# Orbis-Tertius/tiny-ram-halo2

Hardware: AMD Instinct MI355X
Metric: Pallas MSM pairs/s @ 2^24 + Fp NTT elems/s @ 2^22; 1/2/4/8 MI355X (higher is better)
Workload: dtype u255 (255-bit modular integers as 9 x 29/30-bit limbs in i32 / i64 lanes)

## Files before the change

tiny-ram-halo2_amd/csrc/msm.hip:

```cpp
#include <stdlib.h>
#include <string.h>

#include "ctx.h"
#include "devmem.h"
#include "curve_q4.h"
#include "hostcombine.h"
#include "hosthelper.h"
#include "hostplan.h"

namespace trh {

namespace {

using hostplan::MAX_C; using hostplan::MAX_C_FIXED; using hostplan::MSM_TILE; using hostplan::SMALL_C; using hostplan::SMALL_MAX_N;
using hostplan::PART_TILE; using hostplan::BIN_THREADS; using hostplan::BIN_PER_MAX; using hostplan::BIN_CAP_MAX; using hostplan::RANGE_BLOCK;
using hostplan::HEAVY_PIECES; using hostplan::SP_LISTS; using hostplan::SP_CNT; using hostplan::SP_PAD; using hostplan::SP_PARTS; using hostplan::SP_MAX_CHUNK;
using hostplan::num_windows;
static_assert(sizeof(XYZZMem) == hostplan::XYZZ_BYTES && sizeof(XYZZzMem) == hostplan::RAW_POINT_BYTES, "point sizes of the plan's scratch layout");
constexpr u32 SIGN_BIT = 0x80000000u;

template <class SF>
__global__ void __launch_bounds__(256) msm_recode_kernel(const uint4* __restrict__ scalars, size_t n, int mont, int c, int W,
                                                         u32* __restrict__ digits, u32* __restrict__ bin_counts, int k2, u32 nbins, int use_lds, size_t sstride,
                                                         int one_row ,
                                                         const uint4* __restrict__ tails ,
                                                         unsigned char* __restrict__ tile_flags ,
                                                         u32 tile_log, u32 tiles) {
    const size_t z = blockIdx.z;
    const u32 rows = one_row ? 1u : (u32)W;
    scalars += z * sstride * 2; digits += z * (size_t)W * n; bin_counts += z * (size_t)rows * nbins;
    extern __shared__ u32 lhist[];
    const u32 total = rows * nbins;
    if (use_lds) {
        for (u32 k = threadIdx.x; k < total; k += blockDim.x) lhist[k] = 0;
        __syncthreads();
    }
    const u32 mask = (1u << c) - 1u, half = 1u << (c - 1);
    for (size_t i = (size_t)blockIdx.x * blockDim.x + threadIdx.x; i < n; i += (size_t)gridDim.x * blockDim.x) {
        const uint4* src = (tails && i == n - 1) ? tails + 2 * z : scalars + 2 * i;
        uint4 lo = src[0], hi = src[1];
        u32 w[8] = {lo.x, lo.y, lo.z, lo.w, hi.x, hi.y, hi.z, hi.w};
        if (mont) fe_store(fe_from_mont(fe_load<SF>(w)), w);
        u32 carry = 0;
        for (int j = 0; j < W; ++j) {
            u32 raw = (w[0] & mask) + carry;
#pragma unroll
            for (int k = 0; k < 7; ++k) w[k] = (w[k] >> c) | (w[k + 1] << (32 - c));
            w[7] >>= c;
            u32 bucket, sign = 0;
            if (raw > half) { bucket = (1u << c) - raw; carry = 1; sign = SIGN_BIT; }
            else { bucket = raw; carry = 0; }
            digits[(size_t)j * n + i] = bucket ? (bucket | sign) : 0u;
            if (tile_flags) {
                const unsigned long long nz = __ballot(bucket != 0);
                const size_t slot = (size_t)j * n + i;
                const u32 lane = threadIdx.x & 63u;
                if (bucket && ((nz & ((1ull << lane) - 1ull)) == 0ull || (slot & (((size_t)1 << tile_log) - 1)) < 64))
                    tile_flags[z * tiles + (slot >> tile_log)] = 1;
            }
            if (bucket) {
                const u32 bin = (bucket - 1u) >> k2, row = one_row ? 0u : (u32)j;
                if (use_lds) atomicAdd(&lhist[row * nbins + bin], 1u);
                else atomicAdd(&bin_counts[(size_t)row * nbins + bin], 1u);
            }
        }
    }
    if (use_lds) {
        __syncthreads();
        for (u32 k = threadIdx.x; k < total; k += blockDim.x) {
            const u32 v = lhist[k];
            if (v) atomicAdd(&bin_counts[k], v);
        }
    }
}

struct ZeroRanges { uint4* p[4]; u32 n16[4]; };
__global__ void __launch_bounds__(256) msm_zero_ranges_kernel(const ZeroRanges z) {
    const uint4 zero = make_uint4(0, 0, 0, 0);
#pragma unroll
    for (int k = 0; k < 4; ++k)
        for (u32 i = blockIdx.x * blockDim.x + threadIdx.x; i < z.n16[k]; i += gridDim.x * blockDim.x) z.p[k][i] = zero;
}

__global__ void __launch_bounds__(1024) msm_offsets_kernel(u32* __restrict__ counts, u32* __restrict__ starts, u32 nb1, u32* __restrict__ oversize, u32 bin_cap,
                                                           u32* __restrict__ totals ) {
    const size_t z = blockIdx.z;
    counts += z * (size_t)gridDim.x * nb1; starts += z * (size_t)gridDim.x * nb1;
    __shared__ u32 part[1024];
    const int j = blockIdx.x, t = threadIdx.x;
    u32* cnt = counts + (size_t)j * nb1;
    u32* st = starts + (size_t)j * nb1;
    const u32 per = (nb1 + 1023u) / 1024u;
    const u32 lo = t * per < nb1 ? t * per : nb1, hi = (lo + per < nb1) ? lo + per : nb1;
    u32 sum = 0, biggest = 0;
    for (u32 b = lo; b < hi; ++b) { const u32 v = cnt[b]; sum += v; biggest = v > biggest ? v : biggest; }
    if (oversize && biggest > bin_cap) atomicMax(oversize + z * gridDim.x + blockIdx.x, biggest);
    part[t] = sum;
    __syncthreads();
    for (int off = 1; off < 1024; off <<= 1) {
        u32 v = (t >= off) ? part[t - off] : 0;
        __syncthreads();
        part[t] += v;
        __syncthreads();
    }
    if (totals && t == 1023) totals[z * gridDim.x + blockIdx.x] = part[1023];
    u32 run = part[t] - sum;
    for (u32 b = lo; b < hi; ++b) {
        u32 cv = cnt[b];
        st[b] = run;
        cnt[b] = run;
        run += cv;
    }
}

constexpr int PART_THREADS = 1024;
__global__ void __launch_bounds__(PART_THREADS) msm_partition_kernel(const u32* __restrict__ digits, u32* __restrict__ bin_cursor,
                                                                     u32* __restrict__ parted, size_t n, int k2, u32 nbins, int idx_bits,
                                                                     const unsigned char* __restrict__ tile_flags ) {
    const size_t z = blockIdx.z;
    if (tile_flags && !tile_flags[z * gridDim.x + blockIdx.x]) return;
    digits += z * (size_t)gridDim.y * n; parted += z * (size_t)gridDim.y * n; bin_cursor += z * (size_t)gridDim.y * nbins;
    extern __shared__ u32 lds[];
    u32* stage = lds;
    u32* cnt = lds + PART_TILE;
    u32* lbase = cnt + nbins;
    u32* gbase = lbase + nbins;
    __shared__ u32 scan[PART_THREADS];
    const int j = blockIdx.y;
    const size_t t0 = (size_t)blockIdx.x * PART_TILE;
    const size_t t1 = t0 + PART_TILE < n ? t0 + PART_TILE : n;
    const u32* dg = digits + (size_t)j * n;
    for (u32 k = threadIdx.x; k < nbins; k += blockDim.x) cnt[k] = 0;
    __syncthreads();
    constexpr int PER = PART_TILE / PART_THREADS;
    u32 mine[PER];
#pragma unroll
    for (int q = 0; q < PER; ++q) {
        const size_t i = t0 + threadIdx.x + (size_t)q * PART_THREADS;
        mine[q] = i < t1 ? dg[i] : 0u;
    }
#pragma unroll
    for (int q = 0; q < PER; ++q) {
        const u32 b = mine[q] & ~SIGN_BIT;
        if (b) atomicAdd(&cnt[(b - 1u) >> k2], 1u);
    }
    __syncthreads();
    {
        const u32 per = (nbins + PART_THREADS - 1) / PART_THREADS;
        const u32 lo = threadIdx.x * per < nbins ? threadIdx.x * per : nbins, hi = lo + per < nbins ? lo + per : nbins;
        u32 sum = 0;
        for (u32 k = lo; k < hi; ++k) sum += cnt[k];
        scan[threadIdx.x] = sum;
        __syncthreads();
        for (int off = 1; off < PART_THREADS; off <<= 1) {
            const u32 v = ((int)threadIdx.x >= off) ? scan[threadIdx.x - off] : 0;
            __syncthreads();
            scan[threadIdx.x] += v;
            __syncthreads();
        }
        u32 run = scan[threadIdx.x] - sum;
        for (u32 k = lo; k < hi; ++k) {
            const u32 v = cnt[k];
            lbase[k] = run;
            gbase[k] = v ? atomicAdd(&bin_cursor[(size_t)j * nbins + k], v) : 0u;
            run += v;
        }
    }
    __syncthreads();
    for (u32 k = threadIdx.x; k < nbins; k += blockDim.x) cnt[k] = 0;
    __syncthreads();
    const u32 low_mask = (1u << k2) - 1u;
#pragma unroll
    for (int q = 0; q < PER; ++q) {
        const u32 e = mine[q];
        const u32 b = e & ~SIGN_BIT;
        if (b) {
            const u32 bm = b - 1u, bin = bm >> k2;
            const u32 r = atomicAdd(&cnt[bin], 1u);
            stage[lbase[bin] + r] = (u32)(t0 + threadIdx.x + (size_t)q * PART_THREADS) | ((bm & low_mask) << idx_bits) | (e & SIGN_BIT);
        }
    }
    __syncthreads();
    u32* out = parted + (size_t)j * n;
    const u32 wave = threadIdx.x >> 6, lane = threadIdx.x & 63u;
    for (u32 bin = wave; bin < nbins; bin += PART_THREADS / 64) {
        const u32 c = cnt[bin], lb = lbase[bin], gb = gbase[bin];
        for (u32 k = lane; k < c; k += 64) out[gb + k] = stage[lb + k];
    }
}

constexpr int BS_CHUNK = 8192;
constexpr int BS_THREADS = 512;

__device__ __forceinline__ u32 bin_of_position(const u32* __restrict__ bin_ends, u32 nbins, u32 pos) {
    u32 lo = 0, hi = nbins;
    while (lo < hi) {
        const u32 mid = (lo + hi) >> 1;
        if (bin_ends[mid] > pos) hi = mid; else lo = mid + 1;
    }
    return lo;
}

template <bool SCATTER>
__global__ void __launch_bounds__(BS_THREADS) msm_bucket_pass_kernel(const u32* __restrict__ parted, const u32* __restrict__ bin_starts,
                                                                     const u32* __restrict__ bin_ends, u32* __restrict__ bucket_cnt ,
                                                                     u32* __restrict__ sorted, size_t n, int k2, u32 nbins, int idx_bits, u32 nbk,
                                                                     const u32* __restrict__ oversize) {
    const size_t z = blockIdx.z;
    {
        const size_t Wz = gridDim.y;
        parted += z * Wz * n; sorted += z * Wz * n; bin_starts += z * Wz * nbins; bin_ends += z * Wz * nbins;
        bucket_cnt += z * Wz * (nbk + 1);
    }
    if (oversize && oversize[z * gridDim.y + blockIdx.y] == 0u) return;
    __shared__ u32 cnt[128], tbase[128], gbase[128];
    __shared__ u32 stage[SCATTER ? BS_CHUNK : 1];
    const int j = blockIdx.y;
    const u32* bs = bin_starts + (size_t)j * nbins;
    const u32* be = bin_ends + (size_t)j * nbins;
    const u32 total = be[nbins - 1];
    const u32 c0 = blockIdx.x * BS_CHUNK;
    if (c0 >= total) return;
    const u32 c1 = c0 + BS_CHUNK < total ? c0 + BS_CHUNK : total;
    const u32 nsub = 1u << k2, low_mask = nsub - 1u, idx_mask = (1u << idx_bits) - 1u;
    const u32* src = parted + (size_t)j * n;
    u32* dst = sorted + (size_t)j * n;
    u32* bc = bucket_cnt + (size_t)j * (nbk + 1);
    const u32 wave = threadIdx.x >> 6, lane = threadIdx.x & 63u;
    for (u32 bin = bin_of_position(be, nbins, c0); bin < nbins; ++bin) {
        const u32 lo = bs[bin] > c0 ? bs[bin] : c0;
        if (lo >= c1) break;
        const u32 hi = be[bin] < c1 ? be[bin] : c1;
        if (hi <= lo) continue;
        if (hi - lo <= 64u) {
            if (threadIdx.x < hi - lo) {
                const u32 e = src[lo + threadIdx.x];
                u32* cell = &bc[(bin << k2) + ((e >> idx_bits) & low_mask) + 1u];
                if (!SCATTER) atomicAdd(cell, 1u);
                else dst[atomicAdd(cell, 1u)] = (e & idx_mask) | (e & SIGN_BIT);
            }
            continue;
        }
        if (threadIdx.x < 128) cnt[threadIdx.x] = 0;
        __syncthreads();
        for (u32 i = lo + threadIdx.x; i < hi; i += blockDim.x) atomicAdd(&cnt[(src[i] >> idx_bits) & low_mask], 1u);
        __syncthreads();
        if (!SCATTER) {
            if (threadIdx.x < nsub && cnt[threadIdx.x]) atomicAdd(&bc[(bin << k2) + threadIdx.x + 1u], cnt[threadIdx.x]);
        } else {
            if (threadIdx.x == 0) {
                u32 r = 0;
                for (u32 k = 0; k < nsub; ++k) { tbase[k] = r; r += cnt[k]; }
            }
            if (threadIdx.x < nsub) {
                const u32 v = cnt[threadIdx.x];
                gbase[threadIdx.x] = v ? atomicAdd(&bc[(bin << k2) + threadIdx.x + 1u], v) : 0u;
            }
            __syncthreads();
            if (threadIdx.x < 128) cnt[threadIdx.x] = 0;
            __syncthreads();
            for (u32 i = lo + threadIdx.x; i < hi; i += blockDim.x) {
                const u32 e = src[i];
                const u32 sub = (e >> idx_bits) & low_mask;
                const u32 r = atomicAdd(&cnt[sub], 1u);
                stage[tbase[sub] + r] = (e & idx_mask) | (e & SIGN_BIT);
            }
            __syncthreads();
            for (u32 sub = wave; sub < nsub; sub += BS_THREADS / 64) {
                const u32 c = cnt[sub], sb = tbase[sub], gb = gbase[sub];
                for (u32 k = lane; k < c; k += 64) dst[gb + k] = stage[sb + k];
            }
        }
        __syncthreads();
    }
}

template <int PER>
__global__ void __launch_bounds__(BIN_THREADS) msm_bin_sort_kernel(const u32* __restrict__ parted, const u32* __restrict__ bin_starts, const u32* __restrict__ bin_ends,
                                                                   u32* __restrict__ sorted, u32* __restrict__ starts, u32* __restrict__ ends, size_t n, int k2, u32 nbins,
                                                                   int idx_bits, u32 nbk, const u32* __restrict__ oversize) {
    if (oversize[(size_t)blockIdx.z * gridDim.y + blockIdx.y] != 0u) return;
    extern __shared__ u32 bstage[];
    __shared__ u32 cnt[128], tbase[128], wave0_total;
    const size_t z = blockIdx.z, Wz = gridDim.y;
    const int j = blockIdx.y;
    const u32 bin = blockIdx.x;
    const size_t wrow = z * Wz + j;
    const u32 lo = bin_starts[wrow * nbins + bin], hi = bin_ends[wrow * nbins + bin];
    const u32 count = hi - lo;
    const u32 nsub = 1u << k2, low_mask = nsub - 1u, idx_mask = (1u << idx_bits) - 1u;
    const u32* src = parted + wrow * n + lo;
    u32* dst = sorted + wrow * n + lo;
    const u32 lane = threadIdx.x & 63u;
    if (threadIdx.x < 128) cnt[threadIdx.x] = 0;
    __syncthreads();
    u32 mine[PER];
#pragma unroll
    for (int q = 0; q < PER; ++q) {
        const u32 i = threadIdx.x + (u32)q * BIN_THREADS;
        mine[q] = (u32)q * BIN_THREADS < count ? src[i < count ? i : 0u] : 0u;
    }
#pragma unroll
    for (int q = 0; q < PER; ++q)
        if (threadIdx.x + (u32)q * BIN_THREADS < count) atomicAdd(&cnt[(mine[q] >> idx_bits) & low_mask], 1u);
    __syncthreads();
    u32 v = 0, x = 0;
    if (threadIdx.x < 128) {
        v = threadIdx.x < nsub ? cnt[threadIdx.x] : 0u;
        x = v;
#pragma unroll
        for (int off = 1; off < 64; off <<= 1) {
            const u32 y = __shfl_up(x, off, 64);
            if ((int)lane >= off) x += y;
        }
        if (threadIdx.x == 63) wave0_total = x;
    }
    __syncthreads();
    if (threadIdx.x < 128) {
        const u32 excl = x - v + (threadIdx.x >= 64 ? wave0_total : 0u);
        tbase[threadIdx.x] = excl;
        cnt[threadIdx.x] = 0;
        if (threadIdx.x < nsub) {
            const size_t b = wrow * (nbk + 1) + ((size_t)bin << k2) + threadIdx.x + 1u;
            starts[b] = lo + excl;
            ends[b] = lo + excl + v;
        }
        if (bin == 0 && threadIdx.x == 0) { starts[wrow * (nbk + 1)] = 0; ends[wrow * (nbk + 1)] = 0; }
    }
    __syncthreads();
#pragma unroll
    for (int q = 0; q < PER; ++q) {
        if (threadIdx.x + (u32)q * BIN_THREADS < count) {
            const u32 e = mine[q];
            const u32 sub = (e >> idx_bits) & low_mask;
            const u32 r = atomicAdd(&cnt[sub], 1u);
            bstage[tbase[sub] + r] = (e & idx_mask) | (e & SIGN_BIT);
        }
    }
    __syncthreads();
#pragma unroll
    for (int q = 0; q < PER; ++q) {
        const u32 i = threadIdx.x + (u32)q * BIN_THREADS;
        if (i < count) mine[q] = bstage[i];
    }
#pragma unroll
    for (int q = 0; q < PER; ++q) {
        const u32 i = threadIdx.x + (u32)q * BIN_THREADS;
        if (i < count) dst[i] = mine[q];
    }
}

__global__ void __launch_bounds__(RANGE_BLOCK) msm_bucket_block_sums_kernel(const u32* __restrict__ bucket_cnt, u32* __restrict__ block_sums, u32 nbk,
                                                                            const u32* __restrict__ oversize) {
    if (oversize && oversize[(size_t)blockIdx.z * gridDim.y + blockIdx.y] == 0u) return;
    __shared__ u32 part[RANGE_BLOCK / 64];
    const size_t z = blockIdx.z, Wz = gridDim.y;
    const u32 nb1 = nbk + 1, b = blockIdx.x * RANGE_BLOCK + threadIdx.x;
    u32 v = b < nb1 ? bucket_cnt[(z * Wz + blockIdx.y) * nb1 + b] : 0u;
#pragma unroll
    for (int off = 32; off > 0; off >>= 1) v += __shfl_down(v, off, 64);
    if ((threadIdx.x & 63) == 0) part[threadIdx.x >> 6] = v;
    __syncthreads();
    if (threadIdx.x == 0) {
        u32 t = 0;
        for (int k = 0; k < RANGE_BLOCK / 64; ++k) t += part[k];
        block_sums[(z * Wz + blockIdx.y) * gridDim.x + blockIdx.x] = t;
    }
}
__global__ void __launch_bounds__(RANGE_BLOCK) msm_bucket_ranges_kernel(u32* __restrict__ bucket_cnt, const u32* __restrict__ block_sums, u32* __restrict__ starts,
                                                                        u32* __restrict__ ends, u32 nbk, const u32* __restrict__ oversize) {
// ... 666 lines not shown
        if ((int)threadIdx.x < st) sh[threadIdx.x] = xyzzz_add(sh[threadIdx.x], sh[threadIdx.x + st]);
        __syncthreads();
    }
    if (threadIdx.x == 0) store_raw(&part[z * SP_PARTS + g], sh[0]);
}

template <class BF>
__global__ void __launch_bounds__(64) msm_unit_final_kernel(const u32* __restrict__ sp_count, u32 subcap, const XYZZzMem* __restrict__ part, XYZZMem* __restrict__ window_sums,
                                                            int pipeline_ran) {
    const size_t z = blockIdx.x;
    const int unit_mode = sp_count[SP_VOTES] == gridDim.x;
    __shared__ XYZZz<BF> sh[32];
    __shared__ int cls_s;
    if (threadIdx.x == 0) cls_s = sp_classify(sp_count + z * SP_CNT * SP_PAD, SP_PAD, subcap, unit_mode);
    __syncthreads();
    const int cls = cls_s;
    if (cls == SP_CLASS_DENSE) return;
    const u32 t = threadIdx.x;
    if (t < 32) {
        XYZZz<BF> v = xyzzz_identity<BF>();
        if (t < (u32)SP_PARTS) { if (unit_mode) v = load_raw<BF>(&part[z * SP_PARTS + t]); }
        else if (t == (u32)SP_PARTS) { if (pipeline_ran && cls == SP_CLASS_GENERAL) v = xyzzz_from_canonical(load_xyzz<BF>(&window_sums[z])); }
        sh[t] = v;
    }
    __syncthreads();
    for (int st = 16; st > 0; st >>= 1) {
        if ((int)t < st) sh[t] = xyzzz_add(sh[t], sh[t + st]);
        __syncthreads();
    }
    if (t == 0) store_xyzz(&window_sums[z], xyzzz_to_canonical(sh[0]));
}

__global__ void __launch_bounds__(256) msm_sparse_remap_kernel(u32* __restrict__ sorted, const u32* __restrict__ flat, const u32* __restrict__ ends, size_t cap, u32 nbk) {
    const size_t z = blockIdx.y;
    const u32 total = ends[z * (nbk + 1) + nbk];
    sorted += z * cap; flat += z * cap;
    for (u32 k = blockIdx.x * blockDim.x + threadIdx.x; k < total; k += gridDim.x * blockDim.x) {
        const u32 e = sorted[k];
        sorted[k] = flat[e & ~SIGN_BIT] | (e & SIGN_BIT);
    }
}


constexpr u32 SMALL_NBK = 1u << (SMALL_C - 1);
struct SmallBias { u32 w[9]; };

template <class SF, class BF, bool Q4>
__global__ void __launch_bounds__(256) msm_small_kernel(const uint4* __restrict__ bases_z, const uint4* __restrict__ scalars, u32 n, int mont, size_t sstride,
                                                        const uint4* __restrict__ tails, const SmallBias H, XYZZMem* __restrict__ window_sums) {
    __shared__ signed char dig[SMALL_MAX_N];
    __shared__ unsigned short list[SMALL_MAX_N];
    __shared__ u32 hist[SMALL_NBK], cursor[SMALL_NBK], off[SMALL_NBK + 1];
    __shared__ XYZZzMem bsum[SMALL_NBK];
    const u32 j = blockIdx.x, z = blockIdx.y, W = gridDim.x, tid = threadIdx.x;
    scalars += (size_t)z * sstride * 2;
    if (tid < SMALL_NBK) hist[tid] = 0;
    __syncthreads();
    const u32 bit0 = SMALL_C * j, wi = bit0 >> 5, sh = bit0 & 31u;
    for (u32 i = tid; i < n; i += 256) {
        const uint4* src = (tails && i == n - 1) ? tails + 2 * z : scalars + 2 * (size_t)i;
        const uint4 lo = src[0], hi = src[1];
        u32 w[8] = {lo.x, lo.y, lo.z, lo.w, hi.x, hi.y, hi.z, hi.w};
        if (mont) fe_store(fe_from_mont(fe_load<SF>(w)), w);
        u32 v[10];
        u64 cy = 0;
#pragma unroll
        for (int k = 0; k < 8; ++k) { cy += (u64)w[k] + H.w[k]; v[k] = (u32)cy; cy >>= 32; }
        v[8] = (u32)cy + H.w[8]; v[9] = 0;
        u32 a = 0, b = 0;
#pragma unroll
        for (int k = 0; k < 9; ++k) if ((u32)k == wi) { a = v[k]; b = v[k + 1]; }
        const u32 raw = (u32)((((u64)b << 32) | a) >> sh) & ((1u << SMALL_C) - 1u);
        const int d = (int)raw - (int)(SMALL_NBK - 1);
        dig[i] = (signed char)d;
        if (d) atomicAdd(&hist[(d < 0 ? -d : d) - 1], 1u);
    }
    __syncthreads();
    if (tid == 0) {
        u32 run = 0;
        for (u32 b = 0; b < SMALL_NBK; ++b) { off[b] = run; cursor[b] = run; run += hist[b]; }
        off[SMALL_NBK] = run;
    }
    __syncthreads();
    for (u32 i = tid; i < n; i += 256) {
        const int d = dig[i];
        if (d) list[atomicAdd(&cursor[(d < 0 ? -d : d) - 1], 1u)] = (unsigned short)(i | (d < 0 ? 0x8000u : 0u));
    }
    __syncthreads();
    const u32 b = tid >> 4, sl = tid & 15u;
    XYZZz<BF> acc = xyzzz_identity<BF>();
    {
        const u32 start = off[b], cnt = off[b + 1] - start;
        const u32 lo = start + cnt * sl / 16, hi = start + cnt * (sl + 1) / 16;
        for (u32 e = lo; e < hi; ++e) {
            const u32 ent = list[e];
            const uint4* bp = bases_z + (size_t)(ent & 0x7FFFu) * (ZREC / 16);
            const u32 neg = ent >> 15;
            const uint4* yp = bp + 2 + (neg << 1);
            const uint4 qa = bp[0], qb = bp[1], qc = yp[0], qd = yp[1], qt = bp[6];
            AffineZ<BF> p;
            p.x.l[0] = (i32)qa.x; p.x.l[1] = (i32)qa.y; p.x.l[2] = (i32)qa.z; p.x.l[3] = (i32)qa.w;
            p.x.l[4] = (i32)qb.x; p.x.l[5] = (i32)qb.y; p.x.l[6] = (i32)qb.z; p.x.l[7] = (i32)qb.w; p.x.l[8] = (i32)qt.x;
            p.y.l[0] = (i32)qc.x; p.y.l[1] = (i32)qc.y; p.y.l[2] = (i32)qc.z; p.y.l[3] = (i32)qc.w;
            p.y.l[4] = (i32)qd.x; p.y.l[5] = (i32)qd.y; p.y.l[6] = (i32)qd.z; p.y.l[7] = (i32)qd.w; p.y.l[8] = (i32)(neg ? qt.z : qt.y);
            xyzzz_madd(acc, p);
        }
    }
    if constexpr (!Q4) {
        for (int o = 8; o > 0; o >>= 1) {
            const XYZZz<BF> other = shfl_down_point(acc, o, 16);
            if ((int)sl < o) acc = xyzzz_add(acc, other);
        }
        if (sl == 0) store_raw(&bsum[b], acc);
        __syncthreads();
        if (tid >= 64) return;
        XYZZz<BF> v = tid < SMALL_NBK ? load_raw<BF>(&bsum[tid]) : xyzzz_identity<BF>();
        for (int o = 1; o < (int)SMALL_NBK; o <<= 1) {
            const XYZZz<BF> other = shfl_down_point(v, o, 16);
            if (tid < SMALL_NBK && (int)tid + o < (int)SMALL_NBK) v = xyzzz_add(v, other);
        }
        for (int o = SMALL_NBK / 2; o > 0; o >>= 1) {
            const XYZZz<BF> other = shfl_down_point(v, o, 16);
            if ((int)tid < o) v = xyzzz_add(v, other);
        }
        if (tid == 0) store_xyzz(&window_sums[(size_t)z * W + j], xyzzz_to_canonical(v));
    } else {
        __shared__ XYZZzMem pts[SMALL_NBK * 8];
        {
            const XYZZz<BF> other = shfl_down_point(acc, 8, 16);
            if (sl < 8) { acc = xyzzz_add(acc, other); store_raw(&pts[b * 8 + sl], acc); }
        }
        __syncthreads();
        const int q = (int)(tid & 3u);
        const u32 g = tid >> 2;
        auto shfl_fy = [](const Fy<BF>& a, int lanes) {
            Fy<BF> r;
#pragma unroll
            for (int l = 0; l < NLIMBS; ++l) r.l[l] = __shfl_down(a.l[l], lanes);
            return r;
        };
        Fy<BF> v = q4_add(q4_load<BF>(&pts[(g >> 2) * 8 + (g & 3u)], q), q4_load<BF>(&pts[(g >> 2) * 8 + (g & 3u) + 4], q), q);
        v = q4_add(v, q4_select((g & 3u) < 2, shfl_fy(v, 8), fy_zero<BF>()), q);
        v = q4_add(v, q4_select((g & 3u) == 0, shfl_fy(v, 4), fy_zero<BF>()), q);
        if ((g & 3u) == 0) q4_store(&bsum[g >> 2], q, v);
        __syncthreads();
        if (tid >= 64) return;
        v = q4_load<BF>(&bsum[g], q);
        for (int o = 1; o < (int)SMALL_NBK; o <<= 1) v = q4_add(v, q4_select((int)g + o < (int)SMALL_NBK, shfl_fy(v, 4 * o), fy_zero<BF>()), q);
        for (int o = SMALL_NBK / 2; o > 0; o >>= 1) v = q4_add(v, q4_select((int)g < o, shfl_fy(v, 4 * o), fy_zero<BF>()), q);
        if (g == 0) {
            const bool id = q4_is_identity(v);
            uint4* dst = (uint4*)&window_sums[(size_t)z * W + j] + 2 * q;
            if (id) { dst[0] = make_uint4(0, 0, 0, 0); dst[1] = make_uint4(0, 0, 0, 0); }
            else store_fe(dst, fy_to_fe(v));
        }
    }
}

template <class BF> int msm_finish_t(hipStream_t s, u64* out_xyz, size_t batch);
template <class BF> int point_sum_host_t(const u64* pts, size_t count, u64* out);

struct MsmCall {
    const void *bases_dev, *bases_z, *scalars_dev, *tails_dev;
    size_t n, batch, stride;
    int mont;
    hipStream_t s;
    const MsmFixedBase* fb;
    MsmFlags f;
};
template <class SF, class BF> int msm_enqueue_t(const MsmCall& a);

int ensure_host_sums(MsmScratch& m, size_t bytes) {
    if (bytes > m.host_sums_cap) {
        if (m.host_sums) (void)hipHostFree(m.host_sums);
        TRH_HIP_TRY(hipHostMalloc(&m.host_sums, bytes + 4096, hipHostMallocDefault));
        m.host_sums_cap = bytes + 4096;
    }
    return TRH_OK;
}

void set_pending(MsmScratch& m, int curve, int windows, int c, const MsmCall& a, bool timed, bool lean) {
    m.pending_curve = curve; m.pending_windows = windows; m.pending_c = c; m.pending_batch = a.batch; m.pending_stream = a.s; m.pending_owner = nullptr;
    m.pending_in_tile = a.f.in_tile;
    m.ev_valid = timed; m.lean_pending = lean;
}

template <class SF, class BF>
int enqueue_tiled(const MsmCall& a, size_t tiles, size_t len) {
    MsmScratch& m = ctx().msm;
    MsmCall t = a;
    t.batch = 1; t.fb = nullptr; t.f.in_tile = true;
    if (a.f.reserve_only) {
        t.n = t.stride = len; t.tails_dev = nullptr;
        return msm_enqueue_t<SF, BF>(t);
    }
    m.range_tiles = tiles;
    u64 acc[24];
    memset(acc, 0, sizeof(acc));
    int rc = TRH_OK;
    for (size_t off = 0; off < a.n && rc == TRH_OK; off += len) {
        const size_t cur = off + len < a.n ? len : a.n - off;
        const bool last = off + cur == a.n;
        t.bases_dev = (const char*)a.bases_dev + off * 64; t.bases_z = a.bases_z ? (const char*)a.bases_z + off * ZREC : nullptr; t.scalars_dev = (const char*)a.scalars_dev + off * 32;
        t.n = t.stride = cur; t.tails_dev = last ? a.tails_dev : nullptr;
        rc = msm_enqueue_t<SF, BF>(t);
        if (rc != TRH_OK || last) break;
        rc = msm_finish_t<BF>(a.s, acc + 12, 1);
        if (rc == TRH_OK) rc = point_sum_host_t<BF>(acc, 2, acc);
    }
    if (rc != TRH_OK) return rc;
    memcpy(m.tile_sum, acc, 96);
    m.tile_sum_valid = true;
    m.pending_in_tile = false;
    return TRH_OK;
}

template <class SF, class BF>
int enqueue_small(const MsmCall& a) {
    MsmScratch& m = ctx().msm; hipStream_t s = a.s;
    const size_t n = a.n, batch = a.batch;
    const void* bases_z = a.bases_z;
    const int W = num_windows(SMALL_C);
    const size_t hs = batch * W * sizeof(XYZZMem);
    TRH_TRY(m.window_sums.ensure(hs));
    TRH_TRY(ensure_host_sums(m, hs));
    if (!bases_z) TRH_TRY(m.bases_z.ensure(n * ZREC + ZREC));
    if (a.f.reserve_only) return TRH_OK;
    if (!bases_z) {
        hipLaunchKernelGGL((msm_convert_bases_kernel<BF>), dim3((unsigned)((n + 255) / 256)), dim3(256), 0, s, (const uint4*)a.bases_dev, m.bases_z.as<uint4>(), n);
        bases_z = m.bases_z.p;
    }
    SmallBias H{};
    for (int j = 0; j < W; ++j) {
        const u64 v = (u64)(SMALL_NBK - 1) << ((SMALL_C * j) & 31);
        const int k = (SMALL_C * j) >> 5;
        if (k < 9) H.w[k] |= (u32)v;
        if (k + 1 < 9) H.w[k + 1] |= (u32)(v >> 32);
    }
    if (opt().reduce_q4)
        hipLaunchKernelGGL((msm_small_kernel<SF, BF, true>), dim3((unsigned)W, (unsigned)batch), dim3(256), 0, s, (const uint4*)bases_z, (const uint4*)a.scalars_dev, (u32)n, a.mont, a.stride,
                           (const uint4*)a.tails_dev, H, m.window_sums.as<XYZZMem>());
    else
        hipLaunchKernelGGL((msm_small_kernel<SF, BF, false>), dim3((unsigned)W, (unsigned)batch), dim3(256), 0, s, (const uint4*)bases_z, (const uint4*)a.scalars_dev, (u32)n, a.mont, a.stride,
                           (const uint4*)a.tails_dev, H, m.window_sums.as<XYZZMem>());
    TRH_HIP_TRY(hipGetLastError());
    TRH_HIP_TRY(hipMemcpyAsync(m.host_sums, m.window_sums.p, hs, hipMemcpyDeviceToHost, s));
    set_pending(m, BF::ID, W, SMALL_C, a, false, false);
    ++m.small_launches;
    return TRH_OK;
}

struct MsmRun {
    hostplan::MsmPlan p;
    MsmCall a;
    Ctx* c; MsmScratch* m; MsmLane* L;
    const uint4* bz;
    unsigned char* tile_flags;
    u32 *oversize, *totals;
    bool use_bin, lean_sort, sparse_ok, timing;
    const u32* lean_gate;
};
enum { PIPE_PLAIN, PIPE_DENSE, PIPE_COMPACT };
struct MsmChunk {
    size_t b0; unsigned nb; int mode;
    bool compact, zero_fused, bin_sort;
    size_t nse;
    u32 entry_most;
    hostplan::MsmSegments seg;
};

inline int mark(const MsmRun& r, int k) {
    if (r.timing) TRH_HIP_TRY(hipEventRecord(r.m->ev[k], r.a.s));
    return TRH_OK;
}

int reserve_scratch(const MsmRun& r) {
    const hostplan::MsmPlan& p = r.p; MsmScratch& m = *r.m; MsmLane& L = *r.L;
    TRH_TRY(L.digits.ensure(p.entries_bytes()));
    TRH_TRY(L.parted.ensure(p.entries_bytes()));
    TRH_TRY(L.sorted.ensure(p.entries_bytes()));
    TRH_TRY(L.counts.ensure(p.counts_bytes()));
    if (p.adaptive && !r.c->pinned_land) TRH_HIP_TRY(hipHostMalloc(&r.c->pinned_land, 4096, hipHostMallocDefault));
    TRH_TRY(L.bin_starts.ensure(p.bins_bytes(p.chunk)));
    TRH_TRY(L.starts.ensure(p.ranges_bytes(p.chunk)));
    TRH_TRY(L.bucket_cnt.ensure(p.ranges_bytes(p.chunk) + 16));
    TRH_TRY(L.ends.ensure(p.ranges_bytes(p.chunk)));
    TRH_TRY(L.seg_bucket.ensure(p.seg_bucket_bytes()));
    TRH_TRY(L.first.ensure(p.pieces_bytes(p.nseg0)));
    TRH_TRY(L.last.ensure(p.pieces_bytes(p.nseg0)));
    TRH_TRY(L.direct.ensure(p.direct_bytes()));
    TRH_TRY(L.heavy.ensure(p.heavy_bytes(p.chunk, p.heavy_stride0) + 16));
    TRH_TRY(L.buckets.ensure(p.buckets_bytes()));
    TRH_TRY(L.partials.ensure(p.partials_bytes(p.rblocks)));
    if (!r.a.bases_z && !r.a.fb) TRH_TRY(m.bases_z.ensure(p.n * ZREC + ZREC));
    TRH_TRY(m.window_sums.ensure(p.sums_bytes(r.lean_sort)));
    TRH_TRY(ensure_host_sums(m, p.sums_bytes(r.lean_sort)));
    if (r.sparse_ok) {
        TRH_TRY(L.sparse.ensure(p.sparse_bytes()));
        if (!m.sp_host) TRH_HIP_TRY(hipHostMalloc(&m.sp_host, SP_MAX_CHUNK * SP_CNT * 4 + 4 + SP_MAX_CHUNK + 64, hipHostMallocDefault));
    }
    return TRH_OK;
}

template <class SF>
int stage_recode(const MsmRun& r, const MsmChunk& ch) {
    const hostplan::MsmPlan& p = r.p; MsmLane& L = *r.L; hipStream_t s = r.a.s;
    if (ch.zero_fused) {
        auto up16 = [](size_t b) { return (u32)((b + 15) / 16); };
        ZeroRanges zr{};
        zr.p[0] = (uint4*)L.counts.p; zr.n16[0] = up16(p.counts_used());
        zr.p[1] = nullptr; zr.n16[1] = 0u;
        zr.p[2] = (uint4*)L.heavy.p; zr.n16[2] = up16(p.heavy_bytes(ch.nb, p.heavy_stride0));
        zr.p[3] = (uint4*)L.bucket_cnt.p; zr.n16[3] = up16(p.ranges_bytes(ch.nb));
        const u32 most = zr.n16[3] > zr.n16[0] ? zr.n16[3] : zr.n16[0];
        hipLaunchKernelGGL(msm_zero_ranges_kernel, dim3((most + 255) / 256 < 512 ? (most + 255) / 256 : 512), dim3(256), 0, s, zr);
        TRH_HIP_TRY(hipGetLastError());
    }
    if (ch.compact) return TRH_OK;
    if (!ch.zero_fused) TRH_HIP_TRY(hipMemsetAsync(L.counts.p, 0, p.fb ? p.oversize_off() : p.bins_bytes(ch.nb), s));
    const uint4* sc = (const uint4*)((const char*)r.a.scalars_dev + ch.b0 * r.a.stride * 32);
    unsigned gb = (unsigned)((p.n + 255) / 256);
    if (gb > 2048) gb = 2048;
    hipLaunchKernelGGL((msm_recode_kernel<SF>), dim3(gb, 1, ch.nb), dim3(256), p.recode_use_lds ? p.recode_lds : 0, s, sc, p.n, r.a.mont, p.c, p.W,
                       L.digits.as<u32>(), L.counts.as<u32>(), p.k2, p.nbins, p.recode_use_lds, r.a.stride, p.fb ? 1 : 0,
                       r.a.tails_dev ? (const uint4*)r.a.tails_dev + 2 * ch.b0 : nullptr, r.tile_flags, 14u, p.part_tiles);
    static_assert(PART_TILE == 1 << 14, "tile_log of msm_recode_kernel");
    return TRH_OK;
}

int size_segments(const MsmRun& r, MsmChunk& ch, size_t entry_sum) {
    const hostplan::MsmPlan& p = r.p; MsmLane& L = *r.L; hipStream_t s = r.a.s;
    ch.seg = p.seg0();
    bool resize = false;
    if (ch.mode == PIPE_DENSE) {
        ch.seg = hostplan::msm_segments_dense(p, ch.nb);
        resize = true;
    } else if (ch.compact || (p.adaptive && (size_t)ch.nb * p.Ws * 4 <= 4096)) {
        size_t sum = entry_sum;
        u32 most = ch.entry_most;
        if (!ch.compact) {
            u32* ht = (u32*)r.c->pinned_land;
            TRH_HIP_TRY(hipMemcpyAsync(ht, r.totals, (size_t)ch.nb * p.Ws * 4, hipMemcpyDeviceToHost, s));
            TRH_HIP_TRY(hipStreamSynchronize(s));
            sum = 0; most = 0;
            for (size_t q = 0; q < (size_t)ch.nb * p.Ws; ++q) { sum += ht[q]; most = ht[q] > most ? ht[q] : most; }
        }
        ch.seg = hostplan::msm_segments_counted(p, sum, most);
        resize = true;
    }
    if (resize) {
        TRH_TRY(L.first.ensure(p.pieces_bytes(ch.seg.nseg)));
        TRH_TRY(L.last.ensure(p.pieces_bytes(ch.seg.nseg)));
        TRH_TRY(L.heavy.ensure(p.heavy_bytes(p.chunk, ch.seg.heavy_stride)));
    }
    if (ch.zero_fused && (resize || ch.seg.heavy_stride != p.heavy_stride0)) { set_error("msm: internal error: fused zeroing with resized segments"); return TRH_EINVAL; }
    return TRH_OK;
}

template <int P>
void launch_bin_sort(const MsmRun& r, const MsmChunk& ch) {
    const hostplan::MsmPlan& p = r.p; MsmLane& L = *r.L;
    hipLaunchKernelGGL((msm_bin_sort_kernel<P>), dim3(p.nbins, p.Ws, ch.nb), dim3(BIN_THREADS), (size_t)p.bin_cap * 4, r.a.s, L.parted.as<u32>(), L.bin_starts.as<u32>(),
                       L.counts.as<u32>(), L.sorted.as<u32>(), L.starts.as<u32>(), L.ends.as<u32>(), ch.nse, p.k2, p.nbins, p.idx_bits, p.nbk, r.oversize);
}

int stage_sort(const MsmRun& r, MsmChunk& ch, size_t entry_sum) {
    const hostplan::MsmPlan& p = r.p; MsmScratch& m = *r.m; MsmLane& L = *r.L; hipStream_t s = r.a.s;
    const unsigned nb = ch.nb; const int Ws = p.Ws; const size_t nse = ch.nse;
    m.sort_flags = ch.bin_sort ? r.oversize : nullptr; m.sort_flag_count = ch.bin_sort ? nb * (u32)Ws : 0u;
    if (ch.bin_sort && !ch.zero_fused) TRH_HIP_TRY(hipMemsetAsync(r.oversize, 0, p.set_words_bytes(), s));
    hipLaunchKernelGGL(msm_offsets_kernel, dim3(Ws, 1, nb), dim3(1024), 0, s, L.counts.as<u32>(), L.bin_starts.as<u32>(), p.nbins, ch.bin_sort ? r.oversize : nullptr, p.bin_cap,
                       (p.adaptive && ch.mode == PIPE_PLAIN) ? r.totals : nullptr);
    TRH_TRY(size_segments(r, ch, entry_sum));
    if (!ch.zero_fused) TRH_HIP_TRY(hipMemsetAsync(L.heavy.p, 0, p.heavy_bytes(nb, ch.seg.heavy_stride), s));
    hipLaunchKernelGGL(msm_partition_kernel, dim3((unsigned)((nse + PART_TILE - 1) / PART_TILE), Ws, nb), dim3(PART_THREADS), (size_t)PART_TILE * 4 + (size_t)p.nbins * 12, s,
                       L.digits.as<u32>(), L.counts.as<u32>(), L.parted.as<u32>(), nse, p.k2, p.nbins, p.idx_bits, ch.compact ? (const unsigned char*)nullptr : r.tile_flags);
    if (ch.bin_sort) {
        if (p.bin_cap <= 8u * BIN_THREADS) launch_bin_sort<8>(r, ch);
        else if (p.bin_cap <= 18u * BIN_THREADS) launch_bin_sort<18>(r, ch);
        else launch_bin_sort<BIN_PER_MAX>(r, ch);
    }
    if (!r.lean_gate) {
        const dim3 cgrid((unsigned)((nse + BS_CHUNK - 1) / BS_CHUNK), Ws, nb);
        const u32* gate = ch.bin_sort ? r.oversize : nullptr;
        if (!ch.zero_fused) TRH_HIP_TRY(hipMemsetAsync(L.bucket_cnt.p, 0, p.ranges_bytes(nb), s));
        hipLaunchKernelGGL((msm_bucket_pass_kernel<false>), cgrid, dim3(BS_THREADS), 0, s, L.parted.as<u32>(), L.bin_starts.as<u32>(), L.counts.as<u32>(),
                           L.bucket_cnt.as<u32>(), L.sorted.as<u32>(), nse, p.k2, p.nbins, p.idx_bits, p.nbk, gate);
        hipLaunchKernelGGL(msm_bucket_block_sums_kernel, dim3(p.range_blocks, Ws, nb), dim3(RANGE_BLOCK), 0, s, L.bucket_cnt.as<u32>(), L.seg_bucket.as<u32>(), p.nbk, gate);
        hipLaunchKernelGGL(msm_bucket_ranges_kernel, dim3(p.range_blocks, Ws, nb), dim3(RANGE_BLOCK), 0, s, L.bucket_cnt.as<u32>(), L.seg_bucket.as<u32>(), L.starts.as<u32>(),
                           L.ends.as<u32>(), p.nbk, gate);
        hipLaunchKernelGGL((msm_bucket_pass_kernel<true>), cgrid, dim3(BS_THREADS), 0, s, L.parted.as<u32>(), L.bin_starts.as<u32>(), L.counts.as<u32>(),
                           L.bucket_cnt.as<u32>(), L.sorted.as<u32>(), nse, p.k2, p.nbins, p.idx_bits, p.nbk, gate);
    }
    if (ch.compact) {
        unsigned gr = (ch.entry_most + 255) / 256;
        if (gr > 512) gr = 512;
        hipLaunchKernelGGL(msm_sparse_remap_kernel, dim3(gr ? gr : 1, nb), dim3(256), 0, s, L.sorted.as<u32>(), L.digits.as<u32>() + (size_t)p.chunk * p.sp_cap, L.ends.as<u32>(), nse, p.nbk);
    }
    return TRH_OK;
}

template <class BF, int G>
void launch_combine(const MsmRun& r, const MsmChunk& ch) {
    const hostplan::MsmPlan& p = r.p; MsmLane& L = *r.L;
    hipLaunchKernelGGL((msm_combine_kernel<BF, G>), dim3((unsigned)(((size_t)p.nbk * G + 255) / 256), p.Ws, ch.nb), dim3(256), 0, r.a.s, L.starts.as<u32>(), L.ends.as<u32>(),
                       L.first.as<XYZZzMem>(), L.last.as<XYZZzMem>(), L.direct.as<XYZZzMem>(), L.buckets.as<XYZZzMem>(), p.nbk, ch.seg.nseg, ch.seg.seg_len, L.heavy.as<u32>(), ch.seg.heavy_stride,
                       r.lean_gate);
}

template <class BF>
int stage_accumulate(const MsmRun& r, const MsmChunk& ch) {
    const hostplan::MsmPlan& p = r.p; MsmLane& L = *r.L; hipStream_t s = r.a.s;
    const unsigned nb = ch.nb;
    const u32 nbk = p.nbk, nseg = ch.seg.nseg, seg_len = ch.seg.seg_len;
    if (ch.b0 == 0 && !r.a.bases_z && !r.a.fb)
        hipLaunchKernelGGL((msm_convert_bases_kernel<BF>), dim3((unsigned)((p.n + 255) / 256)), dim3(256), 0, s, (const uint4*)r.a.bases_dev, r.m->bases_z.as<uint4>(), p.n);
    hipLaunchKernelGGL((msm_accumulate_seg_kernel<BF>), dim3((nseg + 255) / 256, p.Ws, nb), dim3(256), 0, s, r.bz, L.sorted.as<u32>(),
                       L.ends.as<u32>(), L.first.as<XYZZzMem>(), L.last.as<XYZZzMem>(), L.direct.as<XYZZzMem>(), ch.nse, nbk, nseg, seg_len, r.lean_gate);
    TRH_TRY(mark(r, 5));
    const size_t pieces = ch.compact ? 4 : p.ns / ((size_t)nbk * seg_len);
    if (pieces >= 3 && nbk >= 4 && !ch.compact && opt().reduce_q4 && r.a.f.dense_hint && (size_t)p.Ws * nb <= 8)
        hipLaunchKernelGGL((msm_combine_q4_kernel<BF>), dim3((unsigned)(((size_t)nbk * 4 + 255) / 256), p.Ws, nb), dim3(256), 0, s, L.starts.as<u32>(), L.ends.as<u32>(),
                           L.first.as<XYZZzMem>(), L.last.as<XYZZzMem>(), L.direct.as<XYZZzMem>(), L.buckets.as<XYZZzMem>(), nbk, nseg, seg_len, L.heavy.as<u32>(), ch.seg.heavy_stride,
                           r.lean_gate);
    else if (pieces >= 3 && nbk >= 4) launch_combine<BF, 4>(r, ch);
    else launch_combine<BF, 1>(r, ch);
    hipLaunchKernelGGL((msm_combine_heavy_kernel<BF>), dim3(ch.seg.heavy_blocks, 1, nb), dim3(256), 0, s, L.starts.as<u32>(), L.ends.as<u32>(), L.first.as<XYZZzMem>(),
                       L.last.as<XYZZzMem>(), L.buckets.as<XYZZzMem>(), nbk, nseg, seg_len, L.heavy.as<u32>(), (u32)p.Ws, ch.seg.heavy_stride);
    return TRH_OK;
}

template <class BF>
int stage_reduce(const MsmRun& r, const MsmChunk& ch) {
    const hostplan::MsmPlan& p = r.p; MsmScratch& m = *r.m; MsmLane& L = *r.L; hipStream_t s = r.a.s;
    const unsigned nb = ch.nb; const int Ws = p.Ws; const u32 nbk = p.nbk;
    u32* const sum_flags = (u32*)((char*)m.window_sums.p + p.sum_flags_off());
    const u32 r_tpw = p.tpw, r_slice = p.slice, r_blocks = p.rblocks;
    const int q4_knob = opt().reduce_q4;
    constexpr int q4_lanes_log = 16, q4_sets = 8;
    u32 q4_tpw = r_tpw;
    while (q4_tpw > 1024 && (size_t)q4_tpw * 4 * Ws * nb > ((size_t)1 << q4_lanes_log)) q4_tpw >>= 1;
    if (q4_knob && !ch.compact && (size_t)Ws * nb <= (size_t)q4_sets && q4_tpw >= 64 && (size_t)q4_tpw * 4 * Ws * nb <= ((size_t)1 << q4_lanes_log) && nbk % q4_tpw == 0) {
        const u32 q4_blocks = (q4_tpw + 63) / 64;
        TRH_TRY(L.partials.ensure(p.partials_bytes(q4_blocks)));
        hipLaunchKernelGGL((msm_reduce_q4_kernel<BF>), dim3(q4_blocks, Ws, nb), dim3(256), 0, s, L.buckets.as<XYZZzMem>(), L.partials.as<XYZZzMem>(), nbk, nbk / q4_tpw, q4_tpw);
        hipLaunchKernelGGL((msm_window_sum_q4_kernel<BF>), dim3(Ws, 1, nb), dim3(256), 0, s, L.partials.as<XYZZzMem>(), m.window_sums.as<XYZZMem>() + ch.b0 * Ws, q4_blocks,
                           r.lean_gate, sum_flags, (u32)(nb * Ws));
    } else {
        hipLaunchKernelGGL((msm_reduce_kernel<BF>), dim3(r_blocks, Ws, nb), dim3(256), 0, s, L.buckets.as<XYZZzMem>(), L.partials.as<XYZZzMem>(), nbk, r_slice, r_tpw);
        hipLaunchKernelGGL((msm_window_sum_kernel<BF>), dim3(Ws, 1, nb), dim3(256), 0, s, L.partials.as<XYZZzMem>(), m.window_sums.as<XYZZMem>() + ch.b0 * Ws, r_blocks,
                           r.lean_gate, sum_flags, (u32)(nb * Ws));
    }
    return TRH_OK;
}

template <class SF, class BF>
int run_chunk(const MsmRun& r, size_t b0, unsigned nb, int mode, size_t entry_sum, u32 entry_most) {
    MsmChunk ch{};
    ch.b0 = b0; ch.nb = nb; ch.mode = mode; ch.entry_most = entry_most;
    ch.compact = mode == PIPE_COMPACT;
    ch.nse = ch.compact ? (size_t)r.p.sp_cap : r.p.ns;
    ch.zero_fused = !ch.compact && r.p.batch < 8 && mode != PIPE_DENSE;
    ch.bin_sort = r.use_bin && !ch.compact;
    TRH_TRY(mark(r, 0));
    TRH_TRY(stage_recode<SF>(r, ch));
    TRH_TRY(mark(r, 1));
    TRH_TRY(stage_sort(r, ch, entry_sum));
    TRH_TRY(mark(r, 2));
    TRH_TRY(stage_accumulate<BF>(r, ch));
    TRH_TRY(mark(r, 3));
    TRH_TRY(stage_reduce<BF>(r, ch));
    return mark(r, 4);
}

template <class SF, class BF>
int sparse_chunk(const MsmRun& r, size_t b0, unsigned nb) {
    const hostplan::MsmPlan& p = r.p; MsmScratch& m = *r.m; MsmLane& L = *r.L; hipStream_t s = r.a.s;
    const size_t n = p.n, chunk = p.chunk;
    const u32 sp_subcap = p.sp_subcap, sp_cap = p.sp_cap, nbins = p.nbins;
    const uint4* sc = (const uint4*)((const char*)r.a.scalars_dev + b0 * r.a.stride * 32);
    const uint4* tl = r.a.tails_dev ? (const uint4*)r.a.tails_dev + 2 * b0 : nullptr;
    u32* const sp_count = L.sparse.as<u32>();
    XYZZzMem* const part = (XYZZzMem*)(sp_count + p.sparse_counter_words());
    u32* const digits = L.digits.as<u32>();
    u32* const flat = digits + (size_t)chunk * sp_cap;
    u32* const units = flat + (size_t)chunk * sp_cap;
    u32* const hc = (u32*)m.sp_host;
    u32* const hvotes = hc + SP_MAX_CHUNK * SP_CNT;
    unsigned char* const hd = (unsigned char*)(hvotes + 1);
    TRH_HIP_TRY(hipMemsetAsync(sp_count, 0, (size_t)nb * SP_CNT * SP_PAD * 4, s));
    hipLaunchKernelGGL((msm_sparse_sample_kernel<SF>), dim3(nb), dim3(256), 0, s, sc, n, r.a.mont, p.c, p.W, r.a.stride, tl, sp_count, 2 * sp_cap);
    TRH_HIP_TRY(hipMemcpyAsync(hvotes, sp_count + SP_VOTES, 4, hipMemcpyDeviceToHost, s));
    TRH_HIP_TRY(hipStreamSynchronize(s));
    if (*hvotes != nb) return run_chunk<SF, BF>(r, b0, nb, PIPE_PLAIN, 0, 0);
    TRH_HIP_TRY(hipMemsetAsync(digits, 0, (size_t)nb * sp_cap * 4, s));
    TRH_HIP_TRY(hipMemsetAsync(L.counts.p, 0, (size_t)nb * nbins * 4, s));
    unsigned gbe = (unsigned)((n + 255) / 256);
    if (gbe > 1024) gbe = 1024;
    hipLaunchKernelGGL((msm_sparse_emit_kernel<SF>), dim3(gbe, 1, nb), dim3(256), 0, s, sc, n, r.a.mont, p.c, p.W, r.a.stride, tl, sp_count, digits, flat, units, sp_subcap, L.counts.as<u32>(), p.k2, nbins);
    hipLaunchKernelGGL((msm_unit_sum_kernel<BF>), dim3(SP_PARTS, nb), dim3(256), 0, s, r.bz, sp_count, units, digits, flat, sp_subcap, part);
    TRH_HIP_TRY(hipMemcpy2DAsync(hc, 4, sp_count, SP_PAD * 4, 4, (size_t)nb * SP_CNT, hipMemcpyDeviceToHost, s));
    TRH_HIP_TRY(hipMemcpyAsync(hvotes, sp_count + SP_VOTES, 4, hipMemcpyDeviceToHost, s));
    TRH_HIP_TRY(hipStreamSynchronize(s));
    const int unit_mode = *hvotes == nb;
    size_t sum = 0;
    u32 most = 0, n_general = 0, n_neutral = 0, n_dense = 0;
    for (unsigned z = 0; z < nb; ++z) {
        const int cls = sp_classify(hc + (size_t)z * SP_CNT, 1, sp_subcap, unit_mode);
        hd[z] = (unsigned char)cls;
        size_t cz = 0;
        for (int g = 0; g < SP_LISTS; ++g) cz += hc[(size_t)z * SP_CNT + g];
        if (cls == SP_CLASS_DENSE) {
            ++n_dense;
            if (hc[(size_t)z * SP_CNT] != SP_DENSE) ++n_neutral;
        } else if (cls == SP_CLASS_TINY) {
            if (cz) ++n_neutral;
        } else {
            ++n_general; sum += cz; most = cz > most ? (u32)cz : most;
        }
    }
    const bool run_compact = n_general != 0 && most != 0;
    if (run_compact) {
        if (n_neutral)
            hipLaunchKernelGGL(msm_sparse_neutralise_kernel, dim3(64, nb), dim3(256), 0, s, sp_count, sp_subcap, digits, (size_t)sp_cap, L.counts.as<u32>(), nbins);
        TRH_TRY((run_chunk<SF, BF>(r, b0, nb, PIPE_COMPACT, sum, most)));
    }
    if (n_dense < nb && (unit_mode || !run_compact))
        hipLaunchKernelGGL((msm_unit_final_kernel<BF>), dim3(nb), dim3(64), 0, s, sp_count, sp_subcap, part, m.window_sums.as<XYZZMem>() + b0, run_compact ? 1 : 0);
    for (unsigned z = 0; z < nb;) {
        if (hd[z] != SP_CLASS_DENSE) { ++z; continue; }
        unsigned e = z + 1;
        while (e < nb && hd[e] == SP_CLASS_DENSE) ++e;
        TRH_TRY((run_chunk<SF, BF>(r, b0 + z, e - z, PIPE_DENSE, 0, 0)));
        z = e;
    }
    return TRH_OK;
}

template <class SF, class BF>
int enqueue_pipeline(const MsmCall& a, const hostplan::MsmShape& sh) {
    MsmRun r{};
    r.p = hostplan::msm_plan(sh);
    r.a = a;
    r.c = &ctx(); r.m = &r.c->msm; r.L = &r.m->lane;
    const hostplan::MsmPlan& p = r.p; Ctx& c = *r.c; MsmScratch& m = *r.m; hipStream_t s = a.s;
    const size_t n = a.n, batch = a.batch;
    r.use_bin = p.use_bin_shape && opt().bin_sort;
    r.lean_sort = a.f.dense_hint && !a.f.force_fallback && r.use_bin && batch <= p.chunk && (size_t)batch * p.Ws <= 256 && n != 0 && !(m.lean_off_n == n && m.lean_off_c == p.c);
    r.sparse_ok = opt().sparse && p.sparse_shape_ok && !a.f.dense_hint && !a.f.no_sparse_vote;
    TRH_TRY(reserve_scratch(r));
    if (!(c.attr_done & ATTR_MSM)) {
        TRH_HIP_TRY(hipFuncSetAttribute((const void*)msm_bin_sort_kernel<8>, hipFuncAttributeMaxDynamicSharedMemorySize, 8 * BIN_THREADS * 4));
        TRH_HIP_TRY(hipFuncSetAttribute((const void*)msm_bin_sort_kernel<18>, hipFuncAttributeMaxDynamicSharedMemorySize, 18 * BIN_THREADS * 4));
        TRH_HIP_TRY(hipFuncSetAttribute((const void*)msm_bin_sort_kernel<BIN_PER_MAX>, hipFuncAttributeMaxDynamicSharedMemorySize, BIN_CAP_MAX * 4));
        TRH_HIP_TRY(hipFuncSetAttribute((const void*)msm_partition_kernel, hipFuncAttributeMaxDynamicSharedMemorySize, PART_TILE * 4 + 2048 * 12));
        c.attr_done |= ATTR_MSM;
    }
    if (a.f.reserve_only) return TRH_OK;
    r.bz = a.fb ? (const uint4*)a.fb->table : a.bases_z ? (const uint4*)a.bases_z : m.bases_z.as<uint4>();
    r.tile_flags = a.fb ? (unsigned char*)r.L->counts.p + p.tile_flags_off() : nullptr;
    r.oversize = (u32*)((char*)r.L->counts.p + p.oversize_off());
    r.totals = (u32*)((char*)r.L->counts.p + p.totals_off());
    r.lean_gate = r.lean_sort ? r.oversize : nullptr;
    r.timing = c.timing && batch <= p.chunk && !r.sparse_ok;
    if (r.timing && !m.ev[0]) for (int k = 0; k < 6; ++k) TRH_HIP_TRY(hipEventCreate(&m.ev[k]));

    const size_t hs = p.sums_bytes(r.lean_sort);
    if (!n) {
        TRH_HIP_TRY(hipMemsetAsync(m.window_sums.p, 0, hs, s));
        if (r.timing) for (int k = 0; k <= 5; ++k) TRH_HIP_TRY(hipEventRecord(m.ev[k], s));
    }
    for (size_t b0 = 0; n && b0 < batch; b0 += p.chunk) {
        const unsigned nb = (unsigned)(b0 + p.chunk <= batch ? p.chunk : batch - b0);
        if (r.sparse_ok) TRH_TRY((sparse_chunk<SF, BF>(r, b0, nb)));
        else TRH_TRY((run_chunk<SF, BF>(r, b0, nb, PIPE_PLAIN, 0, 0)));
    }
    TRH_HIP_TRY(hipGetLastError());
    TRH_HIP_TRY(hipMemcpyAsync(m.host_sums, m.window_sums.p, hs, hipMemcpyDeviceToHost, s));
    set_pending(m, BF::ID, p.Ws, p.c, a, r.timing, r.lean_sort);
    if (r.lean_sort) {
        m.retry.bases_dev = a.bases_dev; m.retry.bases_z = a.bases_z; m.retry.scalars_dev = a.scalars_dev; m.retry.tails_dev = a.tails_dev;
        m.retry.n = n; m.retry.batch = batch; m.retry.stride = a.stride; m.retry.mont = a.mont;
        m.retry.has_fb = a.fb != nullptr;
        if (a.fb) m.retry.fb = *a.fb;
        m.retry.flags = a.f;
    }
    return TRH_OK;
}

template <class SF, class BF>
int msm_enqueue_t(const MsmCall& call) {
    Ctx& c = ctx();
    MsmScratch& m = c.msm;
    MsmCall a = call;
    if (a.fb && (a.n == 0 || !msm_fixed_base_fits(a.n, a.fb->c))) a.fb = nullptr;
    if (!a.f.in_tile) m.tile_sum_valid = false;
    if (!a.f.in_tile && !a.f.reserve_only) m.range_tiles = 0;
    m.sort_flags = nullptr; m.sort_flag_count = 0;
    const hostplan::MsmShape sh{a.n, a.batch, a.fb ? a.fb->c : 0, c.window_override, (unsigned)opt().msm_chunk_gb};
    size_t tiles = 0, len = 0;
    switch (hostplan::msm_route(sh, a.f.in_tile, a.f.force_fallback, &tiles, &len)) {
        case hostplan::MSM_ROUTE_TILED: return enqueue_tiled<SF, BF>(a, tiles, len);
        case hostplan::MSM_ROUTE_SMALL: return enqueue_small<SF, BF>(a);
        default: return enqueue_pipeline<SF, BF>(a, sh);
    }
}

template <class BF>
void combine_windows_host(const XYZZMem* ws, int W, int cb, u64* out_xyz) {
    hostcombine::combine_windows<BF>((const uint64_t*)ws, W, cb, (uint64_t*)out_xyz);
}

template <class BF>
int msm_finish_t(hipStream_t s, u64* out_xyz, size_t batch) {
    Ctx& c = ctx();
    MsmScratch& m = c.msm;
    if (m.pending_curve != BF::ID || m.pending_batch != batch || m.pending_stream != s) { set_error("msm_finish: no matching MSM enqueued on this context and stream"); return TRH_EINVAL; }
    const int curve_id = m.pending_curve;
    const bool inner_tile = m.pending_in_tile;
    m.pending_curve = -1;
    TRH_HIP_TRY(hipStreamSynchronize(s));
    if (m.lean_pending) {
        m.lean_pending = false;
        const u32* fl = (const u32*)((const char*)m.host_sums + batch * m.pending_windows * sizeof(XYZZMem));
        bool over = false;
        for (size_t q = 0; q < batch * (size_t)m.pending_windows; ++q) over = over || fl[q] != 0;
        if (over) {
            MsmFlags again = m.retry.flags;
// ... 118 lines not shown
```

Measured before the change: 1.037 billion.

## Specialize MSM recode kernel on window size and mode flags with prefetch

Turns the scalar recode kernel into a template over the window width C and the one-row, LDS-histogram and tile-flag modes, so the per-window digit extraction fully unrolls into constant shifts and the runtime branches disappear. It also prefetches the next scalar before processing the current one, and uses 1024-thread blocks when the LDS histogram is used at full grid, so fewer blocks have to zero and flush the shared histogram. Costs are more template instantiations and larger code. The tile-flags path is now tied to the fallback mode (FLAGS=FB), which assumes tile_flags is only set in that mode.

```diff
diff --git a/tiny-ram-halo2_amd/csrc/msm.hip b/tiny-ram-halo2_amd/csrc/msm.hip
--- a/tiny-ram-halo2_amd/csrc/msm.hip
+++ b/tiny-ram-halo2_amd/csrc/msm.hip
@@ -19,53 +19,85 @@
 static_assert(sizeof(XYZZMem) == hostplan::XYZZ_BYTES && sizeof(XYZZzMem) == hostplan::RAW_POINT_BYTES, "point sizes of the plan's scratch layout");
 constexpr u32 SIGN_BIT = 0x80000000u;
 
-template <class SF>
-__global__ void __launch_bounds__(256) msm_recode_kernel(const uint4* __restrict__ scalars, size_t n, int mont, int c, int W,
-                                                         u32* __restrict__ digits, u32* __restrict__ bin_counts, int k2, u32 nbins, int use_lds, size_t sstride,
-                                                         int one_row ,
+constexpr int RECODE_THREADS_MAX = 1024;
+template <class SF, int C, bool ONE_ROW , bool USE_LDS,
+          bool FLAGS >
+__global__ void __launch_bounds__(RECODE_THREADS_MAX) msm_recode_kernel(const uint4* __restrict__ scalars, size_t n, int mont, int c_arg, int W,
+                                                         u32* __restrict__ digits, u32* __restrict__ bin_counts, int k2, u32 nbins, size_t sstride,
                                                          const uint4* __restrict__ tails ,
-                                                         unsigned char* __restrict__ tile_flags ,
-                                                         u32 tile_log, u32 tiles) {
+                                                         unsigned char* __restrict__ tile_flags, u32 tile_log, u32 tiles) {
     const size_t z = blockIdx.z;
-    const u32 rows = one_row ? 1u : (u32)W;
+    const u32 rows = ONE_ROW ? 1u : (u32)W;
     scalars += z * sstride * 2; digits += z * (size_t)W * n; bin_counts += z * (size_t)rows * nbins;
     extern __shared__ u32 lhist[];
     const u32 total = rows * nbins;
-    if (use_lds) {
+    if (USE_LDS) {
         for (u32 k = threadIdx.x; k < total; k += blockDim.x) lhist[k] = 0;
         __syncthreads();
     }
+    const int c = C ? C : c_arg;
     const u32 mask = (1u << c) - 1u, half = 1u << (c - 1);
-    for (size_t i = (size_t)blockIdx.x * blockDim.x + threadIdx.x; i < n; i += (size_t)gridDim.x * blockDim.x) {
+    const size_t stride = (size_t)gridDim.x * blockDim.x;
+    size_t i = (size_t)blockIdx.x * blockDim.x + threadIdx.x;
+    uint4 lo = make_uint4(0, 0, 0, 0), hi = lo;
+    if (i < n) {
         const uint4* src = (tails && i == n - 1) ? tails + 2 * z : scalars + 2 * i;
-        uint4 lo = src[0], hi = src[1];
+        lo = src[0]; hi = src[1];
+        asm volatile("" : "+v"(lo.x), "+v"(lo.y), "+v"(lo.z), "+v"(lo.w), "+v"(hi.x), "+v"(hi.y), "+v"(hi.z), "+v"(hi.w));
+    }
+    while (i < n) {
         u32 w[8] = {lo.x, lo.y, lo.z, lo.w, hi.x, hi.y, hi.z, hi.w};
+        {
+            const size_t nx = i + stride < n ? i + stride : i;
+            const uint4* src = (tails && nx == n - 1) ? tails + 2 * z : scalars + 2 * nx;
+            lo = src[0]; hi = src[1];
+        }
         if (mont) fe_store(fe_from_mont(fe_load<SF>(w)), w);
         u32 carry = 0;
-        for (int j = 0; j < W; ++j) {
-            u32 raw = (w[0] & mask) + carry;
-#pragma unroll
-            for (int k = 0; k < 7; ++k) w[k] = (w[k] >> c) | (w[k + 1] << (32 - c));
-            w[7] >>= c;
+        u32* dg = digits + i;
+        u32 row = 0;
+        size_t slot = i;
+        auto emit = [&](u32 raw) {
+            raw += carry;
             u32 bucket, sign = 0;
             if (raw > half) { bucket = (1u << c) - raw; carry = 1; sign = SIGN_BIT; }
             else { bucket = raw; carry = 0; }
-            digits[(size_t)j * n + i] = bucket ? (bucket | sign) : 0u;
-            if (tile_flags) {
+            *dg = bucket ? (bucket | sign) : 0u;
+            if (FLAGS) {
                 const unsigned long long nz = __ballot(bucket != 0);
-                const size_t slot = (size_t)j * n + i;
                 const u32 lane = threadIdx.x & 63u;
                 if (bucket && ((nz & ((1ull << lane) - 1ull)) == 0ull || (slot & (((size_t)1 << tile_log) - 1)) < 64))
                     tile_flags[z * tiles + (slot >> tile_log)] = 1;
+                slot += n;
             }
             if (bucket) {
-                const u32 bin = (bucket - 1u) >> k2, row = one_row ? 0u : (u32)j;
-                if (use_lds) atomicAdd(&lhist[row * nbins + bin], 1u);
-                else atomicAdd(&bin_counts[(size_t)row * nbins + bin], 1u);
+                const u32 bin = (bucket - 1u) >> k2;
+                if (USE_LDS) atomicAdd(&lhist[row + bin], 1u);
+                else atomicAdd(&bin_counts[(size_t)row + bin], 1u);
             }
-        }
-    }
-    if (use_lds) {
+            dg += n;
+            if (!ONE_ROW) row += nbins;
+        };
+        if constexpr (C != 0) {
+            constexpr int WC = 255 / C + 1;
+#pragma unroll
+            for (int j = 0; j < WC; ++j) {
+                const int b = j * C, k = b >> 5, s = b & 31;
+                const u32 a0 = k < 8 ? w[k < 8 ? k : 7] : 0u, a1 = (s + C > 32 && k + 1 < 8) ? w[k + 1 < 8 ? k + 1 : 7] : 0u;
+                emit((s ? (a0 >> s) | (a1 << ((32 - s) & 31)) : a0) & mask);
+            }
+        } else {
+            for (int j = 0; j < W; ++j) {
+                const u32 raw = w[0] & mask;
+#pragma unroll
+                for (int k = 0; k < 7; ++k) w[k] = (w[k] >> c) | (w[k + 1] << (32 - c));
+                w[7] >>= c;
+                emit(raw);
+            }
+        }
+        i += stride;
+    }
+    if (USE_LDS) {
         __syncthreads();
         for (u32 k = threadIdx.x; k < total; k += blockDim.x) {
             const u32 v = lhist[k];
@@ -1338,6 +1370,22 @@
     return TRH_OK;
 }
 
+template <class SF, int C, bool FB, bool USE_LDS>
+void launch_recode_mode(const MsmRun& r, const MsmChunk& ch, unsigned gb, const uint4* sc) {
+    const hostplan::MsmPlan& p = r.p; MsmLane& L = *r.L;
+    unsigned threads = 256;
+    if (USE_LDS && gb == 2048) { threads = RECODE_THREADS_MAX; gb = 2048 * 256 / RECODE_THREADS_MAX; }
+    hipLaunchKernelGGL((msm_recode_kernel<SF, C, FB, USE_LDS, FB>), dim3(gb, 1, ch.nb), dim3(threads), USE_LDS ? p.recode_lds : 0, r.a.s, sc, p.n, r.a.mont, p.c, p.W,
+                       L.digits.as<u32>(), L.counts.as<u32>(), p.k2, p.nbins, r.a.stride,
+                       r.a.tails_dev ? (const uint4*)r.a.tails_dev + 2 * ch.b0 : nullptr, r.tile_flags, 14u, p.part_tiles);
+}
+template <class SF, int C>
+void launch_recode(const MsmRun& r, const MsmChunk& ch, unsigned gb, const uint4* sc) {
+    if (r.p.fb) launch_recode_mode<SF, C, true, true>(r, ch, gb, sc);
+    else if (r.p.recode_use_lds) launch_recode_mode<SF, C, false, true>(r, ch, gb, sc);
+    else launch_recode_mode<SF, C, false, false>(r, ch, gb, sc);
+}
+
 template <class SF>
 int stage_recode(const MsmRun& r, const MsmChunk& ch) {
     const hostplan::MsmPlan& p = r.p; MsmLane& L = *r.L; hipStream_t s = r.a.s;
@@ -1357,9 +1405,10 @@
     const uint4* sc = (const uint4*)((const char*)r.a.scalars_dev + ch.b0 * r.a.stride * 32);
     unsigned gb = (unsigned)((p.n + 255) / 256);
     if (gb > 2048) gb = 2048;
-    hipLaunchKernelGGL((msm_recode_kernel<SF>), dim3(gb, 1, ch.nb), dim3(256), p.recode_use_lds ? p.recode_lds : 0, s, sc, p.n, r.a.mont, p.c, p.W,
-                       L.digits.as<u32>(), L.counts.as<u32>(), p.k2, p.nbins, p.recode_use_lds, r.a.stride, p.fb ? 1 : 0,
-                       r.a.tails_dev ? (const uint4*)r.a.tails_dev + 2 * ch.b0 : nullptr, r.tile_flags, 14u, p.part_tiles);
+    if (p.c == 17 && p.W == num_windows(17)) launch_recode<SF, 17>(r, ch, gb, sc);
+    else if (p.c == 16 && p.W == num_windows(16)) launch_recode<SF, 16>(r, ch, gb, sc);
+    else if (p.c == 15 && p.W == num_windows(15)) launch_recode<SF, 15>(r, ch, gb, sc);
+    else launch_recode<SF, 0>(r, ch, gb, sc);
     static_assert(PART_TILE == 1 << 14, "tile_log of msm_recode_kernel");
     return TRH_OK;
 }
```

After: 1.048 billion (median of 6 runs). 1.01x the previous value.
